# xmlyqing00/V-FloodNet

Measured on AMD Instinct MI355X. Metric: segmented frames/sec at 480p, higher is better.
Workload: dtype f32

## Files before the change

include/vfn_winograd6.h:

```cpp
#ifndef VFN_WINOGRAD6_H
#define VFN_WINOGRAD6_H

#ifdef __cplusplus
extern "C" {
#endif

int vfn_winograd6_input_f32(const float* x, int N, int H, int W, int C, int ld_x, int relu, float* V, int rows_pad, void* stream);
int vfn_winograd6_output_f32(const float* Mb, int rows_pad, int N, int H, int W, int Cout, const float* scale, const float* shift,
                             const float* res, int res_ld, int res_mod, int relu_out, float* out, int out_ld, void* stream);

#ifdef __cplusplus
}
#endif

#endif
```

v-floodnet_amd/csrc/conv_winograd.hip:

```cpp
#include "common.h"
#include "conv_internal.h"
#include "../../include/vfn_hip.h"
#include "../../include/vfn_winograd6.h"
#include "../../include/vfn_shortcut_fused.h"

namespace {

__device__ __forceinline__ void bt6(const f32x4 (&v)[6], f32x4 (&t)[6]) {
    t[0] = 4.f * v[0] - 5.f * v[2] + v[4];
    t[1] = -4.f * (v[1] + v[2]) + v[3] + v[4];
    t[2] = 4.f * (v[1] - v[2]) - v[3] + v[4];
    t[3] = -2.f * v[1] - v[2] + 2.f * v[3] + v[4];
    t[4] = 2.f * v[1] - v[2] - 2.f * v[3] + v[4];
    t[5] = 4.f * v[1] - 5.f * v[3] + v[5];
}

template <bool LPOUT = false>
__global__ __launch_bounds__(256)
void winograd_input_kernel(const float* __restrict__ x, int N, int H, int W, int C, int ld_x, int relu, float* __restrict__ V,
                           int rows_pad) {
    const int th = (H + 3) / 4, tw = (W + 3) / 4;
    const int c4n = C / 4;
    const long long total = (long long)N * th * tw * c4n;
    const __amdgpu_buffer_rsrc_t rx = __builtin_amdgcn_make_buffer_rsrc(const_cast<float*>(x), 0, (int)((size_t)N * H * W * ld_x * 4), 0x00020000);
    const float floor_ = relu ? 0.f : -INFINITY;
    for (long long i = vfn_xcd_block(blockIdx.x, gridDim.x) * (long long)blockDim.x + threadIdx.x; i < total; i += (long long)gridDim.x * blockDim.x) {
        const int c4 = (int)(i % c4n);
        const int tile = (int)(i / c4n);
        const int tx = tile % tw, ty = (tile / tw) % th, n = tile / (tw * th);
        f32x4 d[6][6];
#pragma unroll
        for (int a = 0; a < 6; ++a) {
            const int yy = 4 * ty - 1 + a;
#pragma unroll
            for (int b = 0; b < 6; ++b) {
                const int xx = 4 * tx - 1 + b;
                const bool ok = (unsigned)yy < (unsigned)H && (unsigned)xx < (unsigned)W;
                const int off = ok ? (((n * H + yy) * W + xx) * ld_x + c4 * 4) * 4 : 0x7ffffff0;
                d[a][b] = __builtin_bit_cast(f32x4, __builtin_amdgcn_raw_buffer_load_b128(rx, off, 0, 0));
            }
        }
#pragma unroll
        for (int a = 0; a < 6; ++a)
#pragma unroll
            for (int b = 0; b < 6; ++b)
#pragma unroll
                for (int e = 0; e < 4; ++e) d[a][b][e] = vfn_floor_nan(d[a][b][e], floor_);
#pragma unroll
        for (int b = 0; b < 6; ++b) {
            f32x4 v[6], t[6];
#pragma unroll
            for (int a = 0; a < 6; ++a) v[a] = d[a][b];
            bt6(v, t);
#pragma unroll
            for (int a = 0; a < 6; ++a) d[a][b] = t[a];
        }
#pragma unroll
        for (int a = 0; a < 6; ++a) {
            f32x4 t[6];
            bt6(d[a], t);
#pragma unroll
            for (int b = 0; b < 6; ++b) {
                if constexpr (LPOUT) {
                    const vfn_bf16x4 h = {(__bf16)t[b][0], (__bf16)t[b][1], (__bf16)t[b][2], (__bf16)t[b][3]};
                    *reinterpret_cast<vfn_bf16x4*>(reinterpret_cast<__bf16*>(V) + ((size_t)(a * 6 + b) * rows_pad + tile) * C + c4 * 4) = h;
                } else {
                    *reinterpret_cast<f32x4*>(V + ((size_t)(a * 6 + b) * rows_pad + tile) * C + c4 * 4) = t[b];
                }
            }
        }
    }
}

__device__ __forceinline__ void at6(const f32x4 (&m)[6], f32x4 (&y)[4]) {
    const f32x4 s12 = m[1] + m[2], d12 = m[1] - m[2], s34 = m[3] + m[4], d34 = m[3] - m[4];
    y[0] = m[0] + s12 + s34;
    y[1] = d12 + 2.f * d34;
    y[2] = s12 + 4.f * s34;
    y[3] = d12 + 8.f * d34 + m[5];
}

template <bool MASK>
// ... 153 lines not shown
            bt8(d[a], t);
#pragma unroll
            for (int b = 0; b < 8; ++b) __builtin_amdgcn_raw_buffer_store_b64(__builtin_bit_cast(u32x2, t[b]), rv, vo, (a * 8 + b) * comp4, 0);
        }
    }
}

__device__ __forceinline__ void at8(const f32x2 (&m)[8], f32x2 (&y)[6]) {
    const f32x2 s12 = m[1] + m[2], d12 = m[1] - m[2], s34 = m[3] + m[4], d34 = m[3] - m[4], s56 = m[5] + m[6], d56 = m[5] - m[6];
    y[0] = m[0] + s12 + s34 + s56;
    y[1] = d12 + 2.f * d34 + 0.5f * d56;
    y[2] = s12 + 4.f * s34 + 0.25f * s56;
    y[3] = d12 + 8.f * d34 + 0.125f * d56;
    y[4] = s12 + 16.f * s34 + 0.0625f * s56;
    y[5] = d12 + 32.f * d34 + 0.03125f * d56 + m[7];
}

template <bool RES>
__global__ __launch_bounds__(256, RES ? 1 : 2)
void winograd6_output_kernel(const float* __restrict__ Mb, int rows_pad, int N, int H, int W, int Cout,
                             const float* __restrict__ scale, const float* __restrict__ shift, const float* __restrict__ res, int res_ld,
                             int res_mod, int relu_out, float* __restrict__ out, int out_ld) {
    const int th = (H + 5) / 6, tw = (W + 5) / 6;
    const int c2n = Cout / 2;
    const long long total = (long long)N * th * tw * c2n;
    const int npix = N * H * W;
    const __amdgpu_buffer_rsrc_t rm = __builtin_amdgcn_make_buffer_rsrc(const_cast<float*>(Mb), 0, (int)((size_t)64 * rows_pad * Cout * 4), 0x00020000);
    const __amdgpu_buffer_rsrc_t ro = __builtin_amdgcn_make_buffer_rsrc(out, 0, (int)((size_t)npix * out_ld * 4), 0x00020000);
    const __amdgpu_buffer_rsrc_t rr = __builtin_amdgcn_make_buffer_rsrc(const_cast<float*>(res ? res : Mb), 0,
                                                                        res ? (int)((size_t)(res_mod > 0 ? res_mod : npix) * res_ld * 4) : 0, 0x00020000);
    const float floor_ = relu_out ? 0.f : -INFINITY;
    const int comp4 = rows_pad * Cout * 4;
    const long long i = vfn_xcd_block(blockIdx.x, gridDim.x) * (long long)blockDim.x + threadIdx.x;
    if (i >= total) return;
    {
        int iw = (int)i;
        const int mo = ((iw / c2n) * Cout + (iw % c2n) * 2) * 4;
        f32x2 m[8][8];
#pragma unroll
        for (int a = 0; a < 8; ++a)
#pragma unroll
            for (int b = 0; b < 8; ++b) m[a][b] = __builtin_bit_cast(f32x2, __builtin_amdgcn_raw_buffer_load_b64(rm, mo, (a * 8 + b) * comp4, 0));
        f32x2 t[8][6];
#pragma unroll
        for (int a = 0; a < 8; ++a) at8(m[a], t[a]);
        __builtin_amdgcn_sched_barrier(0);
        asm volatile("" : "+v"(iw));
        const int c2 = iw % c2n, tile = iw / c2n;
        const int tx = tile % tw, ty = (tile / tw) % th, n = tile / (tw * th);
        f32x2 sc = {1.f, 1.f}, sh = {0.f, 0.f};
        if (scale) sc = *reinterpret_cast<const f32x2*>(scale + c2 * 2);
        if (shift) sh = *reinterpret_cast<const f32x2*>(shift + c2 * 2);
        const int y0 = 6 * ty, x0 = 6 * tx, row0 = (n * H + y0) * W + x0;
        const int rb = ((row0 - (res_mod > 0 ? (n * H * W) / res_mod * res_mod : 0)) * res_ld + c2 * 2) * 4;
        f32x2 rv[RES ? 6 : 1][RES ? 6 : 1];
        if constexpr (RES) {
#pragma unroll
            for (int a = 0; a < 6; ++a)
#pragma unroll
                for (int b = 0; b < 6; ++b) {
                    const bool ok = y0 + a < H && x0 + b < W;
                    rv[a][b] = __builtin_bit_cast(f32x2, __builtin_amdgcn_raw_buffer_load_b64(rr, ok ? rb + (a * W + b) * res_ld * 4 : 0x7ffffff0, 0, 0));
                }
        }
        const int oo = (row0 * out_ld + c2 * 2) * 4;
#pragma unroll
        for (int b = 0; b < 6; ++b) {
            f32x2 col[8], y[6];
#pragma unroll
            for (int a = 0; a < 8; ++a) col[a] = t[a][b];
            at8(col, y);
#pragma unroll
            for (int a = 0; a < 6; ++a) {
                f32x2 v;
#pragma unroll
                for (int e = 0; e < 2; ++e) v[e] = vfn_floor_nan(y[a][e] * sc[e] + sh[e] + (RES ? rv[a][b][e] : 0.f), floor_);
                const bool ok = y0 + a < H && x0 + b < W;
                __builtin_amdgcn_raw_buffer_store_b64(__builtin_bit_cast(u32x2, v), ro, ok ? oo + (a * W + b) * out_ld * 4 : 0x7ffffff0, 0, 0);
            }
        }
    }
}

__device__ __forceinline__ void a6(const f32x4 (&v)[4], f32x4 (&z)[6]) {
    const f32x4 e = v[0] + v[2], o = v[1] + v[3];
    const f32x4 e4 = v[0] + 4.f * v[2], o8 = 2.f * v[1] + 8.f * v[3];
    z[0] = v[0];
    z[1] = e + o;
    z[2] = e - o;
    z[3] = e4 + o8;
    z[4] = e4 - o8;
    z[5] = v[3];
}

__global__ __launch_bounds__(256)
void winograd_gy_kernel(const float* __restrict__ gy, int N, int H, int W, int C, int ld, float* __restrict__ Z, int rows_pad) {
    const int th = (H + 3) / 4, tw = (W + 3) / 4;
    const int c4n = C / 4;
    const long long total = (long long)N * th * tw * c4n;
    for (long long i = vfn_xcd_block(blockIdx.x, gridDim.x) * (long long)blockDim.x + threadIdx.x; i < total; i += (long long)gridDim.x * blockDim.x) {
        const int c4 = (int)(i % c4n);
        const int tile = (int)(i / c4n);
        const int tx = tile % tw, ty = (tile / tw) % th, n = tile / (tw * th);
        f32x4 t[6][4];
#pragma unroll
        for (int b = 0; b < 4; ++b) {
            f32x4 col[4], z[6];
            const int xx = 4 * tx + b;
#pragma unroll
            for (int a = 0; a < 4; ++a) {
                const int yy = 4 * ty + a;
                f32x4 v = {0.f, 0.f, 0.f, 0.f};
                if (yy < H && xx < W) v = *reinterpret_cast<const f32x4*>(gy + ((size_t)(n * H + yy) * W + xx) * ld + c4 * 4);
                col[a] = v;
            }
            a6(col, z);
#pragma unroll
            for (int a = 0; a < 6; ++a) t[a][b] = z[a];
        }
#pragma unroll
        for (int a = 0; a < 6; ++a) {
            f32x4 z[6];
            a6(t[a], z);
#pragma unroll
            for (int b = 0; b < 6; ++b)
                *reinterpret_cast<f32x4*>(Z + ((size_t)(a * 6 + b) * rows_pad + tile) * C + c4 * 4) = z[b];
        }
    }
}

__device__ __forceinline__ void gt3(const f32x4 (&u)[6], f32x4 (&w)[3]) {
    const f32x4 s12 = u[1] + u[2], d12 = u[2] - u[1], s34 = u[3] + u[4], d34 = u[3] - u[4];
    w[0] = 0.25f * u[0] - (1.f / 6.f) * s12 + (1.f / 24.f) * s34;
    w[1] = (1.f / 6.f) * d12 + (1.f / 12.f) * d34;
    w[2] = -(1.f / 6.f) * s12 + (1.f / 6.f) * s34 + u[5];
}

__global__ __launch_bounds__(256)
void winograd_dw_kernel(const float* __restrict__ dU, int Cout, int Cin, const float* __restrict__ rowscale, float* __restrict__ dw,
                        int accumulate) {
    const int c4n = Cin / 4;
    const long long total = (long long)Cout * c4n;
    const size_t bank = (size_t)Cout * Cin;
    for (long long i = vfn_xcd_block(blockIdx.x, gridDim.x) * (long long)blockDim.x + threadIdx.x; i < total; i += (long long)gridDim.x * blockDim.x) {
        const int c4 = (int)(i % c4n), co = (int)(i / c4n);
        f32x4 t[3][6];
#pragma unroll
        for (int j = 0; j < 6; ++j) {
            f32x4 u[6], w[3];
#pragma unroll
            for (int a = 0; a < 6; ++a) u[a] = *reinterpret_cast<const f32x4*>(dU + (size_t)(a * 6 + j) * bank + (size_t)co * Cin + c4 * 4);
            gt3(u, w);
#pragma unroll
            for (int a = 0; a < 3; ++a) t[a][j] = w[a];
        }
        const float sc = rowscale ? rowscale[co] : 1.f;
#pragma unroll
        for (int a = 0; a < 3; ++a) {
            f32x4 w[3];
            gt3(t[a], w);
#pragma unroll
            for (int b = 0; b < 3; ++b) {
                f32x4* o = reinterpret_cast<f32x4*>(dw + ((size_t)co * 9 + a * 3 + b) * Cin + c4 * 4);
                f32x4 v = w[b] * sc;
                if (accumulate) v += *o;
                *o = v;
// ... 20 lines not shown
    const float* U;
    const float* scale;
    const float* shift;
    int C, a_ld, cout_pad, relu_in, relu_mid, stride, H, W, Ho, Wo, pix;
};

template <int BM, int BN, int WM, int WN, int PD, bool CONV = false, bool LP = false>
__global__ __launch_bounds__(WM * WN * 64)
void wino_gemm_kernel(const wino_gemm_args p) {
    constexpr bool DUAL = false;
    constexpr wino_dual_args q2{};
#include "wino_gemm_body.inc"
}

template <int BM, int BN, int WM, int WN, int PD>
__global__ __launch_bounds__(WM * WN * 64)
void wino_gemm_dual_kernel(const wino_gemm_args p, const wino_dual_args q2) {
    constexpr bool DUAL = true, CONV = true, LP = false;
#include "wino_gemm_body.inc"
}

template <int BM, int BN, int WM, int WN, int PD, bool CONV, bool LP, bool DUAL = false>
int launch_wino_gemm(const wino_gemm_args& a, int wgs, hipStream_t s, const wino_dual_args* dual = nullptr) {
    constexpr size_t lds = 2 * (size_t)(BM + BN) * 32 * sizeof(float);
    static const bool lds_ready = [] {
        if constexpr (DUAL) return vfn_allow_lds(&wino_gemm_dual_kernel<BM, BN, WM, WN, PD>, lds);
        else return vfn_allow_lds(&wino_gemm_kernel<BM, BN, WM, WN, PD, CONV, LP>, lds);
    }();
    (void)lds_ready;
    wino_gemm_args p = a;
    p.mtiles = (a.rows_pad + BM - 1) / BM;
    p.ntiles = (a.Cout + BN - 1) / BN;
    const int total = p.comps * p.mtiles * p.ntiles;
    int grid = wgs > 0 ? wgs : 512;
    if (grid > total) grid = total;
    grid = (grid + 7) / 8 * 8;
    if constexpr (DUAL)
        hipLaunchKernelGGL((wino_gemm_dual_kernel<BM, BN, WM, WN, PD>), dim3(grid), dim3(WM * WN * 64), lds, s, p, *dual);
    else
        hipLaunchKernelGGL((wino_gemm_kernel<BM, BN, WM, WN, PD, CONV, LP>), dim3(grid), dim3(WM * WN * 64), lds, s, p);
    return vfn_check_launch();
}

constexpr int kWinoTile[4][4] = {{128, 128, 4, 2}, {64, 128, 2, 4}, {128, 64, 4, 2}, {64, 64, 2, 2}};
constexpr int kWinoCfgs = 8;

constexpr int kWinoDualCfgs = 4;

template <bool CONV, bool LP, bool DUAL = false>
int launch_wino_cfg(const wino_gemm_args& a, int cfg, int wgs, hipStream_t s, const wino_dual_args* dual = nullptr) {
    return vfn_dispatch<DUAL ? kWinoDualCfgs : kWinoCfgs>(cfg, [&](auto id) -> int {
        constexpr int c = decltype(id)::value;
        constexpr const int* t = kWinoTile[c & 3];
        return launch_wino_gemm<t[0], t[1], t[2], t[3], 1 + (c >> 2), CONV, LP, DUAL>(a, wgs, s, dual);
    });
}

constexpr int kWinoTile32[2][4] = {{32, 128, 1, 4}, {32, 64, 1, 2}};
constexpr int kWinoCfgs32 = 8;

inline const int* wino_tile_of(int cfg) { return cfg < kWinoCfgs ? kWinoTile[cfg & 3] : kWinoTile32[cfg & 1]; }
inline bool wino_cfg32_ok(int cfg) { return cfg >= kWinoCfgs && cfg < kWinoCfgs + kWinoCfgs32 && (cfg & 3) < 2; }

int launch_wino_cfg32(const wino_gemm_args& a, int cfg, int wgs, hipStream_t s) {
    switch (cfg - kWinoCfgs) {
        case 0: return launch_wino_gemm<32, 128, 1, 4, 1, false, false>(a, wgs, s);
        case 1: return launch_wino_gemm<32, 64, 1, 2, 1, false, false>(a, wgs, s);
        case 4: return launch_wino_gemm<32, 128, 1, 4, 2, false, false>(a, wgs, s);
        case 5: return launch_wino_gemm<32, 64, 1, 2, 2, false, false>(a, wgs, s);
    }
    return VFN_ERR_ARG;
}

inline bool tensors_fit_32bit(int N, int H, int W, int ld, int res_ld, int mask_ld, int res_mod) {
    const long long px = (long long)N * H * W;
    return px * ld * 4 < 0x7fffff00LL && (res_mod > 0 ? (long long)res_mod : px) * res_ld * 4 < 0x7fffff00LL && px * mask_ld * 4 < 0x7fffff00LL;
}

inline int grid_of(long long total) {
    long long b = (total + 255) / 256;
    return (int)(b < 16384 ? (b ? b : 1) : 16384);
}

}

extern "C" int vfn_winograd_tiles(int N, int H, int W) { return N * ((H + 3) / 4) * ((W + 3) / 4); }

extern "C" int vfn_winograd_input_f32(const float* x, int N, int H, int W, int C, int ld_x, int relu, float* V, int rows_pad, void* stream) {
    if (!x || !V || N < 1 || H < 1 || W < 1 || C < 4 || C % 4 || ld_x < C || ld_x % 4 || rows_pad < vfn_winograd_tiles(N, H, W)) return VFN_ERR_ARG;
    const long long total = (long long)vfn_winograd_tiles(N, H, W) * (C / 4);
    if (!tensors_fit_32bit(N, H, W, ld_x, 0, 0, 0)) return VFN_ERR_ARG;
    hipLaunchKernelGGL(winograd_input_kernel<false>, dim3(grid_of(total)), dim3(256), 0, (hipStream_t)stream, x, N, H, W, C, ld_x, relu, V, rows_pad);
    return vfn_check_launch();
}

extern "C" int vfn_winograd_output_f32(const float* Mb, int rows_pad, int N, int H, int W, int Cout, const float* scale, const float* shift,
                                       const float* res, int res_ld, int res_mod, int relu_out, float* out, int out_ld, void* stream) {
    if (!Mb || !out || N < 1 || H < 1 || W < 1 || Cout < 4 || Cout % 4 || out_ld < Cout || out_ld % 4 || (res && res_ld % 4) ||
        rows_pad < vfn_winograd_tiles(N, H, W)) return VFN_ERR_ARG;
    const long long total = (long long)vfn_winograd_tiles(N, H, W) * (Cout / 4);
    if (!tensors_fit_32bit(N, H, W, out_ld, res ? res_ld : 0, 0, res_mod)) return VFN_ERR_ARG;
    hipLaunchKernelGGL(winograd_output_kernel<false>, dim3(grid_of(total)), dim3(256), 0, (hipStream_t)stream, Mb, rows_pad, N, H, W, Cout, scale, shift,
                       res, res_ld, res_mod, relu_out, out, out_ld, (const float*)nullptr, 0, 0);
    return vfn_check_launch();
}

extern "C" int vfn_winograd6_input_f32(const float* x, int N, int H, int W, int C, int ld_x, int relu, float* V, int rows_pad, void* stream) {
    if (!x || !V || N < 1 || H < 1 || W < 1 || C < 4 || C % 4 || ld_x < C || ld_x % 4 || rows_pad < winograd6_tiles(N, H, W)) return VFN_ERR_ARG;
    if (!tensors_fit_32bit(N, H, W, ld_x, 0, 0, 0) || (long long)64 * rows_pad * C * 4 >= 0x7fffff00LL) return VFN_ERR_ARG;
    hipLaunchKernelGGL(winograd6_input_kernel, dim3(((long long)rows_pad * (C / 2) + 255) / 256), dim3(256), 0, (hipStream_t)stream, x, N, H, W, C, ld_x, relu,
                       V, rows_pad);
    return vfn_check_launch();
}

extern "C" int vfn_winograd6_output_f32(const float* Mb, int rows_pad, int N, int H, int W, int Cout, const float* scale, const float* shift,
                                        const float* res, int res_ld, int res_mod, int relu_out, float* out, int out_ld, void* stream) {
    if (!Mb || !out || N < 1 || H < 1 || W < 1 || Cout < 4 || Cout % 4 || out_ld < Cout || out_ld % 4 || (res && res_ld % 4) ||
        rows_pad < winograd6_tiles(N, H, W) || res_mod < 0 || (res && res_mod % (H * W))) return VFN_ERR_ARG;
    if (!tensors_fit_32bit(N, H, W, out_ld, res ? res_ld : 0, 0, res_mod) || (long long)64 * rows_pad * Cout * 4 >= 0x7fffff00LL) return VFN_ERR_ARG;
    const dim3 grid(((long long)winograd6_tiles(N, H, W) * (Cout / 2) + 255) / 256);
    if (res)
        hipLaunchKernelGGL(winograd6_output_kernel<true>, grid, dim3(256), 0, (hipStream_t)stream, Mb, rows_pad, N, H, W, Cout, scale, shift, res, res_ld,
                           res_mod, relu_out, out, out_ld);
    else
        hipLaunchKernelGGL(winograd6_output_kernel<false>, grid, dim3(256), 0, (hipStream_t)stream, Mb, rows_pad, N, H, W, Cout, scale, shift, res, res_ld,
                           res_mod, relu_out, out, out_ld);
    return vfn_check_launch();
}

extern "C" int vfn_winograd_output_masked_f32(const float* Mb, int rows_pad, int N, int H, int W, int Cout, const float* res, int res_ld,
                                              const float* mask, int mask_ld, int mask_after, float* out, int out_ld, void* stream) {
    if (!Mb || !out || N < 1 || H < 1 || W < 1 || Cout < 4 || Cout % 4 || out_ld < Cout || out_ld % 4 || (res && res_ld % 4) ||
        (mask && mask_ld % 4) || rows_pad < vfn_winograd_tiles(N, H, W)) return VFN_ERR_ARG;
    const long long total = (long long)vfn_winograd_tiles(N, H, W) * (Cout / 4);
    if (!tensors_fit_32bit(N, H, W, out_ld, res ? res_ld : 0, mask ? mask_ld : 0, 0)) return VFN_ERR_ARG;
    if (mask)
        hipLaunchKernelGGL(winograd_output_kernel<true>, dim3(grid_of(total)), dim3(256), 0, (hipStream_t)stream, Mb, rows_pad, N, H, W, Cout,
                           (const float*)nullptr, (const float*)nullptr, res, res_ld, 0, 0, out, out_ld, mask, mask_ld, mask_after);
    else
        hipLaunchKernelGGL(winograd_output_kernel<false>, dim3(grid_of(total)), dim3(256), 0, (hipStream_t)stream, Mb, rows_pad, N, H, W, Cout,
                           (const float*)nullptr, (const float*)nullptr, res, res_ld, 0, 0, out, out_ld, (const float*)nullptr, 0, 0);
    return vfn_check_launch();
}

extern "C" int vfn_winograd_gy_f32(const float* gy, int N, int H, int W, int C, int ld, float* Z, int rows_pad, void* stream) {
    if (!gy || !Z || N < 1 || H < 1 || W < 1 || C < 4 || C % 4 || ld < C || ld % 4 || rows_pad < vfn_winograd_tiles(N, H, W)) return VFN_ERR_ARG;
    const long long total = (long long)vfn_winograd_tiles(N, H, W) * (C / 4);
    hipLaunchKernelGGL(winograd_gy_kernel, dim3(grid_of(total)), dim3(256), 0, (hipStream_t)stream, gy, N, H, W, C, ld, Z, rows_pad);
    return vfn_check_launch();
}

extern "C" int vfn_winograd_dw_f32(const float* dU, int Cout, int Cin, const float* rowscale, float* dw, int accumulate, void* stream) {
    if (!dU || !dw || Cout < 1 || Cin < 4 || Cin % 4) return VFN_ERR_ARG;
    hipLaunchKernelGGL(winograd_dw_kernel, dim3(grid_of((long long)Cout * (Cin / 4))), dim3(256), 0, (hipStream_t)stream, dU, Cout, Cin, rowscale,
                       dw, accumulate);
    return vfn_check_launch();
}

extern "C" int vfn_winograd_gemm_f32(const float* V, const float* U, float* Mb, int comps, int rows_pad, int C, int Cout, int cout_pad, int cfg,
                                     int wgs, void* stream) {
    if (!V || !U || !Mb || comps < 1 || rows_pad < 1 || C < 32 || C % 32 || Cout < 1 || cout_pad < Cout || cfg < 0 ||
        (cfg >= kWinoCfgs && !wino_cfg32_ok(cfg))) return VFN_ERR_ARG;
    const int bm = wino_tile_of(cfg)[0], bn = wino_tile_of(cfg)[1];
    if (rows_pad % bm || cout_pad < (Cout + bn - 1) / bn * bn) return VFN_ERR_ARG;
    if ((long long)comps * rows_pad * C * 4 >= 0x7fffff00LL || (long long)comps * cout_pad * C * 4 >= 0x7fffff00LL) return VFN_ERR_ARG;
    wino_gemm_args a{V, U, Mb, comps, rows_pad, C, Cout, cout_pad, 0, 0, 0, 0, 0, 0, 0, 0, nullptr, nullptr, nullptr};
    if (cfg >= kWinoCfgs) return launch_wino_cfg32(a, cfg, wgs, (hipStream_t)stream);
    return launch_wino_cfg<false, false>(a, cfg, wgs, (hipStream_t)stream);
}

extern "C" int vfn_conv1x1_persistent_f32(const vfn_conv_desc* d, int cfg, int wgs, void* stream) {
    if (!d || !d->in || !d->w || !d->out || cfg < 0 || cfg >= kWinoCfgs) return VFN_ERR_ARG;
    if (d->KH != 1 || d->KW != 1 || d->stride != 1 || d->pad != 0 || d->mask || d->in_lp || d->out_lp || d->w_packed || d->ksplit > 1 ||
        d->w_batch_rows || d->Cin % 32 || d->in_ld % 4 || d->M < 1 || d->M != d->N * d->H * d->W) return VFN_ERR_ARG;
    const int bn = kWinoTile[cfg & 3][1];
    if (d->cout_pad < (d->Cout + bn - 1) / bn * bn) return VFN_ERR_ARG;
    const long long lim = 0x7fffff00LL;
    if ((long long)d->M * d->in_ld * 4 >= lim || (long long)d->M * d->out_ld * 4 >= lim || (long long)d->cout_pad * d->Cin * 4 >= lim ||
        (d->res && (long long)(d->res_mod > 0 ? d->res_mod : d->M) * d->res_ld * 4 >= lim)) return VFN_ERR_ARG;
    wino_gemm_args a{d->in, d->w, d->out, 1, d->M, d->Cin, d->Cout, d->cout_pad, 0, 0,
                     d->in_ld, d->out_ld, d->res ? d->res_ld : 0, d->res_mod, d->relu_in, d->relu_out, d->scale, d->shift, d->res};
    return launch_wino_cfg<true, false>(a, cfg, wgs, (hipStream_t)stream);
}

extern "C" int vfn_conv1x1_shortcut_fused_f32(const vfn_conv_desc* sc, const vfn_conv_desc* d, int cfg, int wgs, void* stream) {
    if (!sc || !d || !sc->in || !sc->w || !d->in || !d->w || !d->out || cfg < 0 || cfg >= kWinoDualCfgs) return VFN_ERR_ARG;
    for (const vfn_conv_desc* l : {sc, d})
        if (l->KH != 1 || l->KW != 1 || l->pad != 0 || l->mask || l->in_lp || l->out_lp || l->w_packed || l->ksplit > 1 || l->w_batch_rows ||
            l->res || l->Cin < 32 || l->Cin % 32 || l->in_ld < l->Cin || l->in_ld % 4 || l->N < 1 || l->H < 1 || l->W < 1) return VFN_ERR_ARG;
    if (d->stride != 1 || (sc->stride != 1 && sc->stride != 2)) return VFN_ERR_ARG;
    if (d->M < 1 || d->M != d->N * d->H * d->W || sc->Ho != (sc->H - 1) / sc->stride + 1 || sc->Wo != (sc->W - 1) / sc->stride + 1 ||
        sc->M != sc->N * sc->Ho * sc->Wo || sc->M != d->M || sc->Cout != d->Cout || d->Cout < 1 || d->out_ld < d->Cout) return VFN_ERR_ARG;
    const int bn = kWinoTile[cfg & 3][1];
    const int need = (d->Cout + bn - 1) / bn * bn;
    if (d->cout_pad < need || sc->cout_pad < need) return VFN_ERR_ARG;
    const long long lim = 0x7fffff00LL, pix2 = (long long)sc->N * sc->H * sc->W;
    if (pix2 * sc->in_ld * 4 >= lim || (long long)d->M * d->in_ld * 4 >= lim || (long long)d->M * d->out_ld * 4 >= lim ||
        (long long)d->cout_pad * d->Cin * 4 >= lim || (long long)sc->cout_pad * sc->Cin * 4 >= lim) return VFN_ERR_ARG;
    wino_gemm_args a{d->in, d->w, d->out, 1, d->M, d->Cin, d->Cout, d->cout_pad, 0, 0,
                     d->in_ld, d->out_ld, 0, 0, d->relu_in, d->relu_out, d->scale, d->shift, nullptr};
    const wino_dual_args a2{sc->in, sc->w, sc->scale, sc->shift, sc->Cin, sc->in_ld, sc->cout_pad, sc->relu_in, sc->relu_out, sc->stride,
                            sc->H, sc->W, sc->Ho, sc->Wo, (int)pix2};
    return launch_wino_cfg<true, false, true>(a, cfg, wgs, (hipStream_t)stream, &a2);
}

extern "C" int vfn_winograd_input_bf16(const float* x, int N, int H, int W, int C, int ld_x, int relu, void* V, int rows_pad, void* stream) {
    if (!x || !V || N < 1 || H < 1 || W < 1 || C < 4 || C % 4 || ld_x < C || ld_x % 4 || rows_pad < vfn_winograd_tiles(N, H, W)) return VFN_ERR_ARG;
    const long long total = (long long)vfn_winograd_tiles(N, H, W) * (C / 4);
    if (!tensors_fit_32bit(N, H, W, ld_x, 0, 0, 0)) return VFN_ERR_ARG;
// ... 16 lines not shown
```

v-floodnet_amd/ops.py:

```python
import ctypes as C
import os

import torch

from . import _lib
from ._lib import ptr, stream, check, ConvDesc


_cfg_tiles = None


def conv_cfg_tiles():
    global _cfg_tiles
    if _cfg_tiles is None:
        L = _lib.lib()
        out = []
        for c in range(L.vfn_conv_cfg_count()):
            bm, bn = C.c_int(), C.c_int()
            L.vfn_conv_cfg_tile(c, C.byref(bm), C.byref(bn))
            out.append((bm.value, bn.value))
        _cfg_tiles = tuple(out)
    return _cfg_tiles


# ... 322 lines not shown
                                                    (c >> 3) * 128, stream()), 'vfn_winograd_gemm_bf16')
            return
        if mode != 0 or rows <= 0:
            raise RuntimeError('the persistent GEMM takes an f32 (or plain-bf16) Winograd-domain descriptor (w_batch_rows)')
        check(_lib.lib().vfn_winograd_gemm_f32(desc.inp, desc.w, desc.out, desc.M // rows, rows, desc.Cin, desc.Cout, desc.cout_pad, c & 7,
                                               (c >> 3) * 128, stream()), 'vfn_winograd_gemm_f32')
        return
    name = _CONV_FN[int(mode)]
    check(getattr(_lib.lib(), name)(C.byref(desc), cfg, stream()), name)


def conv_cfg_name(cfg, mode=0, _cache={}):
    cfg = int(cfg)
    if is_thin3x3_cfg(cfg):
        return f'conv_thin3x3_kernel<{thin3x3_cfg_info(cfg)[0]}>'
    if cfg >= WINO_GEMM_CFG0:
        bm, bn, wm, wn, pd, _ = persistent_cfg_info(cfg)
        return f'wino_gemm_kernel<{bm}, {bn}, {wm}, {wn}, {pd}, {"true" if cfg >= PCONV_CFG0 else "false"}, {"true" if mode == 1 else "false"}>'
    if mode not in _cache:
        _cache[mode] = conv_cfg_names(mode)
    return _cache[mode][cfg]


def conv2d_nhwc(x, wp, cout, kh, kw, stride, pad, scale=None, shift=None, res=None,
                relu_in=False, relu_out=False, cfg=3, out=None, mode=0):
    N, H, W, _ = x.shape
    Ho = (H + 2 * pad - kh) // stride + 1
    Wo = (W + 2 * pad - kw) // stride + 1
    if out is None:
        out = torch.empty(N, Ho, Wo, cout, device=x.device, dtype=torch.float32)
    d = make_conv_desc(x, wp, cout, kh, kw, stride, pad, out, scale, shift, res, relu_in, relu_out)
    if mode == 0 and conv_cfg_kind(cfg) == 2:
        set_streamk(d, *streamk_scratch(x.device))
    conv2d_launch(d, cfg, mode)
    return out


_WINO_G = torch.tensor([[1 / 4, 0, 0], [-1 / 6, -1 / 6, -1 / 6], [-1 / 6, 1 / 6, -1 / 6], [1 / 24, 1 / 12, 1 / 6], [1 / 24, -1 / 12, 1 / 6], [0, 0, 1]],
                       dtype=torch.float64)
WINO_ROW_MULT = 256
_WINO_KROT = int(os.environ.get('VFN_KROT', '0'))


def pack_winograd_weight(w):
    cout, cin = w.shape[0], w.shape[1]
    assert tuple(w.shape[2:]) == (3, 3)
    g = w.detach().double().cpu()
    U = torch.einsum('ia,ocab,jb->ijoc', _WINO_G, g, _WINO_G)
    cp = (cout + 255) // 256 * 256
    out = torch.zeros(36, cp, cin, dtype=torch.float32)
    out[:, :cout] = U.reshape(36, cout, cin).float()
    return out.reshape(36 * cp, cin).contiguous()


def winograd_rows(N, H, W):
    t = N * ((H + 3) // 4) * ((W + 3) // 4)
    return (t + WINO_ROW_MULT - 1) // WINO_ROW_MULT * WINO_ROW_MULT


_WINO6_G = torch.tensor([[1, 0, 0], [-2 / 9, -2 / 9, -2 / 9], [-2 / 9, 2 / 9, -2 / 9], [1 / 90, 1 / 45, 2 / 45], [1 / 90, -1 / 45, 2 / 45],
                         [32 / 45, 16 / 45, 8 / 45], [32 / 45, -16 / 45, 8 / 45], [0, 0, 1]], dtype=torch.float64)
WINO6_ROW_MULT = 64


def pack_winograd6_weight(w):
    cout, cin = w.shape[0], w.shape[1]
    assert tuple(w.shape[2:]) == (3, 3)
    g, G = w.detach().double().cpu(), _WINO6_G
    col = lambda k: G[:, k].view(8, 1)
    tmp = (col(0) * g[:, :, None, 0, :] + col(1) * g[:, :, None, 1, :]) + col(2) * g[:, :, None, 2, :]
    U = (tmp[..., 0, None] * G[:, 0] + tmp[..., 1, None] * G[:, 1]) + tmp[..., 2, None] * G[:, 2]
    cp = (cout + 255) // 256 * 256
    out = torch.zeros(64, cp, cin, dtype=torch.float32)
    out[:, :cout] = U.permute(2, 3, 0, 1).reshape(64, cout, cin).float()
    return out.reshape(64 * cp, cin).contiguous()


def winograd6_tiles(N, H, W):
    return N * ((H + 5) // 6) * ((W + 5) // 6)


def winograd6_rows(N, H, W):
    return (winograd6_tiles(N, H, W) + WINO6_ROW_MULT - 1) // WINO6_ROW_MULT * WINO6_ROW_MULT


def pack_winograd_weight_bf16(w):
    return pack_winograd_weight(w).to(torch.bfloat16).contiguous()


def winograd_input(x, V, rows_pad, relu, N=None, H=None, W=None, cin=None, ld_x=None, tile=4):
    if N is None:
        N, H, W = x.shape[0], x.shape[1], x.shape[2]
    cin = cin if cin is not None else x.shape[-1]
    ld_x = ld_x if ld_x is not None else x.shape[-1]
    if tile == 6:
        check(_lib.lib().vfn_winograd6_input_f32(ptr(x), N, H, W, cin, ld_x, int(relu), ptr(V), rows_pad, stream()), 'vfn_winograd6_input_f32')
        return
    if V.dtype == torch.bfloat16:
        check(_lib.lib().vfn_winograd_input_bf16(ptr(x), N, H, W, cin, ld_x, int(relu), ptr(V), rows_pad, stream()), 'vfn_winograd_input_bf16')
        return
    check(_lib.lib().vfn_winograd_input_f32(ptr(x), N, H, W, cin, ld_x, int(relu), ptr(V), rows_pad, stream()), 'vfn_winograd_input_f32')


def winograd_output(Mb, rows_pad, out, N, H, W, cout, scale, shift, res, res_ld, res_mod, relu_out, out_ld=None, tile=4):
    name = 'vfn_winograd6_output_f32' if tile == 6 else 'vfn_winograd_output_f32'
    check(getattr(_lib.lib(), name)(ptr(Mb), rows_pad, N, H, W, cout, ptr(scale), ptr(shift), ptr(res), int(res_ld), int(res_mod),
                                    int(relu_out), ptr(out), out_ld if out_ld is not None else out.shape[-1], stream()), name)


def make_winograd_gemm_desc(V, U, Mb, rows_pad, cin, cout, comps=36):
    d = make_conv_desc(V, U, cout, 1, 1, 1, 0, Mb, None, None, None, False, False, cin=cin, in_ld=cin, out_ld=cout, N=1, H=1, W=comps * rows_pad)
    d.cout_pad = U.shape[0] // comps
    d.w_batch_rows = rows_pad
    d.k_rot = _WINO_KROT
    return d


def winograd_gemm(V, U, Mb, rows_pad, cin, cout, cfg=0, wgs=0, comps=36):
    check(_lib.lib().vfn_winograd_gemm_f32(ptr(V), ptr(U), ptr(Mb), comps, rows_pad, cin, cout, U.shape[0] // comps, int(cfg), int(wgs), stream()),
          'vfn_winograd_gemm_f32')


def conv2d_winograd(x, w, scale=None, shift=None, res=None, relu_in=False, relu_out=False, cfg=2, res_mod=0, tile=4):
    N, H, W, cin = x.shape
    cout = w.shape[0]
    if tile == 6:
        comps, rows, tiles = 64, winograd6_rows(N, H, W), winograd6_tiles(N, H, W)
        U = pack_winograd6_weight(w).to(x.device)
    else:
        comps, rows, tiles = 36, winograd_rows(N, H, W), vfn_winograd_tiles(N, H, W)
        U = pack_winograd_weight(w).to(x.device)
    V = torch.empty(comps * rows, cin, device=x.device, dtype=torch.float32)
    Mb = torch.empty(comps * rows, cout, device=x.device, dtype=torch.float32)
    out = torch.empty(N, H, W, cout, device=x.device, dtype=torch.float32)
    if rows > tiles and tile != 6:
        V.view(comps, rows, cin)[:, tiles:].zero_()
    assert x.stride(3) == 1 and x.stride(1) == W * x.stride(2) and x.stride(0) == H * x.stride(1)
    winograd_input(x, V, rows, relu_in, ld_x=x.stride(2), tile=tile)
    d = make_winograd_gemm_desc(V, U, Mb, rows, cin, cout, comps)
    if conv_cfg_kind(cfg) == 2:
        set_streamk(d, *streamk_scratch(x.device))
    conv2d_launch(d, cfg, 0)
    winograd_output(Mb, rows, out, N, H, W, cout, scale, shift, res, res.shape[-1] if res is not None else 0, res_mod, relu_out, tile=tile)
    return out


def vfn_winograd_tiles(N, H, W):
    return N * ((H + 3) // 4) * ((W + 3) // 4)


def make_stem_desc(frame, mask, w, scale, shift, out, mean, std, N, H0, W0, pad, Hp, Wp):
    from ._lib import StemDesc
    d = StemDesc()
    d.frame, d.mask, d.w, d.scale, d.shift, d.out = ptr(frame), ptr(mask), ptr(w), ptr(scale), ptr(shift), ptr(out)
    for i in range(3):
        d.mean[i] = float(mean[i])
        d.std[i] = float(std[i])
    d.N, d.cin = N, (5 if mask is not None else 3)
    d.H0, d.W0 = H0, W0
    d.pad_top, d.pad_left = pad[2], pad[0]
    d.Hp, d.Wp, d.Ho, d.Wo = Hp, Wp, Hp // 2, Wp // 2
    return d


def stem_launch(desc):
    check(_lib.lib().vfn_stem_conv7x7_f32(C.byref(desc), stream()), 'vfn_stem_conv7x7_f32')
# ... 483 lines not shown
```

Measured before the change: 170.5.

## Split Winograd F(6,3) transforms across 8 threads per tile via LDS

Adds input and output transform kernels for the 8x8 Winograd path where each tile is handled by 8 threads. Each thread does one 1D transform pass, the partial results are exchanged through shared memory, and the second pass follows. The aim is to cut per-thread register pressure and raise parallelism compared with one thread transforming a whole tile. A shape-based auto selector keeps the old kernel for a couple of specific output shapes, and an env variable or API can force either form, at the cost of an extra LDS round-trip and a barrier.

```diff
diff --git a/include/vfn_winograd6.h b/include/vfn_winograd6.h
--- a/include/vfn_winograd6.h
+++ b/include/vfn_winograd6.h
@@ -8,6 +8,8 @@
 int vfn_winograd6_input_f32(const float* x, int N, int H, int W, int C, int ld_x, int relu, float* V, int rows_pad, void* stream);
 int vfn_winograd6_output_f32(const float* Mb, int rows_pad, int N, int H, int W, int Cout, const float* scale, const float* shift,
                              const float* res, int res_ld, int res_mod, int relu_out, float* out, int out_ld, void* stream);
+int vfn_winograd6_form(int N, int H, int W, int C, int is_output, int has_res);
+int vfn_winograd6_force_form(int form);
 
 #ifdef __cplusplus
 }
diff --git a/v-floodnet_amd/csrc/conv_winograd.hip b/v-floodnet_amd/csrc/conv_winograd.hip
--- a/v-floodnet_amd/csrc/conv_winograd.hip
+++ b/v-floodnet_amd/csrc/conv_winograd.hip
@@ -1,3 +1,6 @@
+#include <atomic>
+#include <cstdlib>
+#include <cstring>
 #include "common.h"
 #include "conv_internal.h"
 #include "../../include/vfn_hip.h"
@@ -317,6 +320,119 @@
     }
 }
 
+constexpr int kW6Oob = 0x7ffffff0;
+
+__device__ __forceinline__ f32x2 w6_load(__amdgpu_buffer_rsrc_t r, int voff, int soff) {
+    return __builtin_bit_cast(f32x2, __builtin_amdgcn_raw_buffer_load_b64(r, voff, soff, 0));
+}
+__device__ __forceinline__ void w6_store(f32x2 v, __amdgpu_buffer_rsrc_t r, int voff, int soff) {
+    __builtin_amdgcn_raw_buffer_store_b64(__builtin_bit_cast(u32x2, v), r, voff, soff, 0);
+}
+template <bool RES>
+__device__ __forceinline__ f32x2 w6_epilogue(const f32x2& y, const f32x2& sc, const f32x2& sh, const f32x2& r, float floor_) {
+    f32x2 v;
+#pragma unroll
+    for (int e = 0; e < 2; ++e) v[e] = vfn_floor_nan(y[e] * sc[e] + sh[e] + (RES ? r[e] : 0.f), floor_);
+    return v;
+}
+
+template <bool RELU>
+__global__ __launch_bounds__(256)
+void winograd6_input_split_kernel(const float* __restrict__ x, int N, int H, int W, int C, int ld_x, float* __restrict__ V, int rows_pad) {
+    __shared__ f32x2 lds[64 * 32];
+    const int th = (H + 5) / 6, tw = (W + 5) / 6, tiles = N * th * tw;
+    const int c2n = C / 2, groups = (c2n + 31) / 32;
+    const __amdgpu_buffer_rsrc_t rx = __builtin_amdgcn_make_buffer_rsrc(const_cast<float*>(x), 0, (int)((size_t)N * H * W * ld_x * 4), 0x00020000);
+    const __amdgpu_buffer_rsrc_t rv = __builtin_amdgcn_make_buffer_rsrc(V, 0, (int)((size_t)64 * rows_pad * C * 4), 0x00020000);
+    const int comp4 = rows_pad * C * 4;
+    const int blk = (int)vfn_xcd_block(blockIdx.x, gridDim.x);
+    const int tile = blk / groups, cg = blk - tile * groups;
+    const int cp = threadIdx.x & 31, j = threadIdx.x >> 5;
+    const int c2 = cg * 32 + cp;
+    const bool live = c2 < c2n;
+    const int vo = live ? (tile * C + c2 * 2) * 4 + j * 8 * comp4 : kW6Oob;
+    if (tile >= tiles) {
+#pragma unroll
+        for (int b = 0; b < 8; ++b) w6_store(f32x2{0.f, 0.f}, rv, live ? vo + b * comp4 : kW6Oob, 0);
+        return;
+    }
+    const int tx = tile % tw, ty = (tile / tw) % th, n = tile / (tw * th);
+    const int y0 = 6 * ty - 1, x0 = 6 * tx - 1;
+    const bool colok = live && (unsigned)(x0 + j) < (unsigned)W;
+    const int px4 = ld_x * 4;
+    f32x2 v[8], t[8];
+#pragma unroll
+    for (int a = 0; a < 8; ++a) {
+        const bool ok = colok && (unsigned)(y0 + a) < (unsigned)H;
+        v[a] = w6_load(rx, ok ? ((n * H + y0 + a) * W + x0 + j) * px4 + c2 * 8 : kW6Oob, 0);
+    }
+    if constexpr (RELU) {
+#pragma unroll
+        for (int a = 0; a < 8; ++a)
+#pragma unroll
+            for (int e = 0; e < 2; ++e) v[a][e] = vfn_floor_nan(v[a][e], 0.f);
+    }
+    bt8(v, t);
+#pragma unroll
+    for (int a = 0; a < 8; ++a) lds[(a * 8 + j) * 32 + cp] = t[a];
+    __syncthreads();
+#pragma unroll
+    for (int b = 0; b < 8; ++b) v[b] = lds[(j * 8 + b) * 32 + cp];
+    bt8(v, t);
+#pragma unroll
+    for (int b = 0; b < 8; ++b) w6_store(t[b], rv, live ? vo + b * comp4 : kW6Oob, 0);
+}
+
+template <bool RES>
+__global__ __launch_bounds__(256)
+void winograd6_output_split_kernel(const float* __restrict__ Mb, int rows_pad, int N, int H, int W, int Cout,
+                                   const float* __restrict__ scale, const float* __restrict__ shift, const float* __restrict__ res, int res_ld,
+                                   int res_mod, int relu_out, float* __restrict__ out, int out_ld) {
+    __shared__ f32x2 lds[64 * 32];
+    const int th = (H + 5) / 6, tw = (W + 5) / 6;
+    const int c2n = Cout / 2, groups = (c2n + 31) / 32;
+    const int npix = N * H * W;
+    const __amdgpu_buffer_rsrc_t rm = __builtin_amdgcn_make_buffer_rsrc(const_cast<float*>(Mb), 0, (int)((size_t)64 * rows_pad * Cout * 4), 0x00020000);
+    const __amdgpu_buffer_rsrc_t ro = __builtin_amdgcn_make_buffer_rsrc(out, 0, (int)((size_t)npix * out_ld * 4), 0x00020000);
+    const __amdgpu_buffer_rsrc_t rr = __builtin_amdgcn_make_buffer_rsrc(const_cast<float*>(RES ? res : Mb), 0,
+                                                                        RES ? (int)((size_t)(res_mod > 0 ? res_mod : npix) * res_ld * 4) : 0, 0x00020000);
+    const float floor_ = relu_out ? 0.f : -INFINITY;
+    const int comp4 = rows_pad * Cout * 4;
+    const int blk = (int)vfn_xcd_block(blockIdx.x, gridDim.x);
+    const int tile = blk / groups, cg = blk - tile * groups;
+    const int cp = threadIdx.x & 31, j = threadIdx.x >> 5;
+    const int c2 = cg * 32 + cp;
+    const bool live = c2 < c2n;
+    const int tx = tile % tw, ty = (tile / tw) % th, n = tile / (tw * th);
+    const int y0 = 6 * ty, x0 = 6 * tx, row0 = (n * H + y0) * W + x0;
+    const bool colok = live && j < 6 && x0 + j < W;
+    f32x2 m[8], t[6];
+    const int mo = (tile * Cout + c2 * 2) * 4 + j * 8 * comp4;
+#pragma unroll
+    for (int b = 0; b < 8; ++b) m[b] = w6_load(rm, live ? mo + b * comp4 : kW6Oob, 0);
+    f32x2 rv[6];
+    if constexpr (RES) {
+        const int rb = ((row0 + j - (res_mod > 0 ? (n * H * W) / res_mod * res_mod : 0)) * res_ld + c2 * 2) * 4;
+#pragma unroll
+        for (int a = 0; a < 6; ++a) rv[a] = w6_load(rr, colok && y0 + a < H ? rb + a * W * res_ld * 4 : kW6Oob, 0);
+    }
+    f32x2 sc = {1.f, 1.f}, sh = {0.f, 0.f};
+    if (scale && live) sc = *reinterpret_cast<const f32x2*>(scale + c2 * 2);
+    if (shift && live) sh = *reinterpret_cast<const f32x2*>(shift + c2 * 2);
+    at8(m, t);
+#pragma unroll
+    for (int b = 0; b < 6; ++b) lds[(j * 8 + b) * 32 + cp] = t[b];
+    __syncthreads();
+    if (j >= 6) return;
+#pragma unroll
+    for (int a = 0; a < 8; ++a) m[a] = lds[(a * 8 + j) * 32 + cp];
+    at8(m, t);
+    const int oo = ((row0 + j) * out_ld + c2 * 2) * 4;
+#pragma unroll
+    for (int a = 0; a < 6; ++a)
+        w6_store(w6_epilogue<RES>(t[a], sc, sh, rv[a], floor_), ro, colok && y0 + a < H ? oo + a * W * out_ld * 4 : kW6Oob, 0);
+}
+
 __device__ __forceinline__ void a6(const f32x4 (&v)[4], f32x4 (&z)[6]) {
     const f32x4 e = v[0] + v[2], o = v[1] + v[3];
     const f32x4 e4 = v[0] + 4.f * v[2], o8 = 2.f * v[1] + 8.f * v[3];
@@ -503,6 +619,34 @@
     return (int)(b < 16384 ? (b ? b : 1) : 16384);
 }
 
+std::atomic<int> g_wino6_forced{-1};
+
+int wino6_env_form() {
+    static const int v = [] {
+        const char* e = getenv("VFN_WINO6_XFORM");
+        if (!e || !*e || !strcmp(e, "auto")) return -1;
+        const int k = atoi(e);
+        return k >= 0 && k <= 2 ? k : -1;
+    }();
+    return v;
+}
+
+int wino6_auto_form(int tiles, int C, bool is_output, bool has_res) {
+    static const int keep0_out[][2] = {{45, 640}, {1440, 256}};
+    if (is_output && !has_res)
+        for (const auto& k : keep0_out)
+            if (tiles == k[0] && C == k[1]) return 0;
+    return 2;
+}
+
+int wino6_form(int N, int H, int W, int C, int is_output, int has_res) {
+    const int forced = g_wino6_forced.load(std::memory_order_relaxed);
+    const int want = forced >= 0 ? forced : wino6_env_form();
+    if (want == 0 || want == 1) return 0;
+    if (want == 2) return 2;
+    return wino6_auto_form(winograd6_tiles(N, H, W), C, is_output != 0, has_res != 0);
+}
+
 }
 
 extern "C" int vfn_winograd_tiles(int N, int H, int W) { return N * ((H + 3) / 4) * ((W + 3) / 4); }
@@ -529,9 +673,27 @@
 extern "C" int vfn_winograd6_input_f32(const float* x, int N, int H, int W, int C, int ld_x, int relu, float* V, int rows_pad, void* stream) {
     if (!x || !V || N < 1 || H < 1 || W < 1 || C < 4 || C % 4 || ld_x < C || ld_x % 4 || rows_pad < winograd6_tiles(N, H, W)) return VFN_ERR_ARG;
     if (!tensors_fit_32bit(N, H, W, ld_x, 0, 0, 0) || (long long)64 * rows_pad * C * 4 >= 0x7fffff00LL) return VFN_ERR_ARG;
-    hipLaunchKernelGGL(winograd6_input_kernel, dim3(((long long)rows_pad * (C / 2) + 255) / 256), dim3(256), 0, (hipStream_t)stream, x, N, H, W, C, ld_x, relu,
-                       V, rows_pad);
+    const hipStream_t s = (hipStream_t)stream;
+    if (wino6_form(N, H, W, C, 0, 0) == 2) {
+        const dim3 grid((long long)rows_pad * ((C / 2 + 31) / 32));
+        if (relu) hipLaunchKernelGGL(winograd6_input_split_kernel<true>, grid, dim3(256), 0, s, x, N, H, W, C, ld_x, V, rows_pad);
+        else hipLaunchKernelGGL(winograd6_input_split_kernel<false>, grid, dim3(256), 0, s, x, N, H, W, C, ld_x, V, rows_pad);
+    } else {
+        hipLaunchKernelGGL(winograd6_input_kernel, dim3(((long long)rows_pad * (C / 2) + 255) / 256), dim3(256), 0, s, x, N, H, W, C, ld_x, relu, V,
+                           rows_pad);
+    }
     return vfn_check_launch();
+}
+
+extern "C" int vfn_winograd6_form(int N, int H, int W, int C, int is_output, int has_res) {
+    if (N < 1 || H < 1 || W < 1 || C < 4 || C % 4) return -1;
+    return wino6_form(N, H, W, C, is_output, has_res);
+}
+
+extern "C" int vfn_winograd6_force_form(int form) {
+    if (form < -1 || form > 3) return VFN_ERR_ARG;
+    g_wino6_forced.store(form, std::memory_order_relaxed);
+    return VFN_OK;
 }
 
 extern "C" int vfn_winograd6_output_f32(const float* Mb, int rows_pad, int N, int H, int W, int Cout, const float* scale, const float* shift,
@@ -539,13 +701,13 @@
     if (!Mb || !out || N < 1 || H < 1 || W < 1 || Cout < 4 || Cout % 4 || out_ld < Cout || out_ld % 4 || (res && res_ld % 4) ||
         rows_pad < winograd6_tiles(N, H, W) || res_mod < 0 || (res && res_mod % (H * W))) return VFN_ERR_ARG;
     if (!tensors_fit_32bit(N, H, W, out_ld, res ? res_ld : 0, 0, res_mod) || (long long)64 * rows_pad * Cout * 4 >= 0x7fffff00LL) return VFN_ERR_ARG;
-    const dim3 grid(((long long)winograd6_tiles(N, H, W) * (Cout / 2) + 255) / 256);
-    if (res)
-        hipLaunchKernelGGL(winograd6_output_kernel<true>, grid, dim3(256), 0, (hipStream_t)stream, Mb, rows_pad, N, H, W, Cout, scale, shift, res, res_ld,
-                           res_mod, relu_out, out, out_ld);
-    else
-        hipLaunchKernelGGL(winograd6_output_kernel<false>, grid, dim3(256), 0, (hipStream_t)stream, Mb, rows_pad, N, H, W, Cout, scale, shift, res, res_ld,
-                           res_mod, relu_out, out, out_ld);
+    const long long tiles = winograd6_tiles(N, H, W);
+    const int form = wino6_form(N, H, W, Cout, 1, res != nullptr);
+    const dim3 grid(form == 2 ? tiles * ((Cout / 2 + 31) / 32) : (tiles * (Cout / 2) + 255) / 256);
+    auto* kernel = form == 2 ? (res ? winograd6_output_split_kernel<true> : winograd6_output_split_kernel<false>)
+                             : (res ? winograd6_output_kernel<true> : winograd6_output_kernel<false>);
+    hipLaunchKernelGGL(kernel, grid, dim3(256), 0, (hipStream_t)stream, Mb, rows_pad, N, H, W, Cout, scale, shift, res, res_ld, res_mod, relu_out, out,
+                       out_ld);
     return vfn_check_launch();
 }
 
diff --git a/v-floodnet_amd/ops.py b/v-floodnet_amd/ops.py
--- a/v-floodnet_amd/ops.py
+++ b/v-floodnet_amd/ops.py
@@ -428,6 +428,10 @@
 
 def winograd6_rows(N, H, W):
     return (winograd6_tiles(N, H, W) + WINO6_ROW_MULT - 1) // WINO6_ROW_MULT * WINO6_ROW_MULT
+
+
+def winograd6_form(N, H, W, C, is_output, has_res):
+    return _lib.lib().vfn_winograd6_form(N, H, W, C, int(is_output), int(has_res))
 
 
 def pack_winograd_weight_bf16(w):
```

New measurement: 172.7, median of 6. 1.3% higher.
